# Chthi/Ofighters

Hardware: AMD Instinct MI355X
Metric: arena-steps/sec (env.step+obs+policy fwd) at 4096 arenas, 1/2/4/8 MI355X (higher is better)
Workload: dtype f32; 1 GPU; 4096 arenas x 8 ships per GPU, random-bot actions + step + 2D obs rasterise (u8 maps) + bi-head policy forward for 8 ship(s)/arena, trunk shared per arena (BASELINE configs[3]); arenas_per_gpu=4096, ships=8, laser_cap=512, episode_ticks=200, parallelism=arena-sharded x1, RCCL all-reduce of episodic scores only, laser_overflow=0, last_episode_score_sum=70993, last_episode_arenas=4096

## Files before the change

### ofighters_amd/csrc/ofx_head.hip

```cpp
#include "ofx_head.h"
#include "ofx_lowp.h"
#include "ofx_diag.h"
#include <stdlib.h>


typedef float f32x4 __attribute__((ext_vector_type(4)));
typedef float f32x2 __attribute__((ext_vector_type(2)));
#define HD_PS 400
constexpr int HC4_ZERO = 800;
constexpr int HC4_COL = 816, HC4_CPITCH = 416;
constexpr int HC4_STRIDE = HC4_COL + 2 * HC4_CPITCH + 16;
__device__ __forceinline__ int hc4_at(int ln, int t) { return ln < 2 ? ln * 400 + t : HC4_COL + (ln - 2) * HC4_CPITCH + t; }
__device__ __forceinline__ int hc4_pad(int k) { return k < 16 ? HC4_ZERO + k : k < 32 ? HC4_COL + 400 + k - 16 : HC4_COL + HC4_CPITCH + 400 + k - 32; }

__device__ __forceinline__ void hc4_zero_block(const HeadParams2 &p, int tid, int threads) {
  if (blockIdx.x == 0)
    for (int e = tid; e < HC4_STRIDE; e += threads) p.c4[(size_t)p.S * HC4_STRIDE + e] = 0.f;
}

__device__ __forceinline__ float hd_max_raw(float x, float floor) {
  float pinf;
  asm("s_mov_b32 %0, 0x7f800000" : "=s"(pinf));
  return __builtin_amdgcn_fmed3f(x, floor, pinf);
}
// ... 182 lines not shown
    float acc = 0.f;
    if (!isc || (t > 0 && t < 399)) {
      const int d0 = side ? 2 : 0;
#pragma unroll
      for (int d1 = 0; d1 < 3; d1++)
#pragma unroll
        for (int ci = 0; ci < 8; ci++) {
          const int tap = isc ? d1 * 3 + d0 : d0 * 3 + d1;
          acc += p.w4raw[tap * 8 + ci] * hf_up(u3l + ln * 1600 + ci, 8, 200, t + d1 - 1, p.legacy);
        }
      if (!isc && (t == 0 || t == 399)) {
        const int cl = t ? 3 : 2, dx = t ? 2 : 0;
        for (int dy = 0; dy < 3; dy++) {
          if (dy == d0) continue;
          const int yy = (side ? 399 : 0) + dy - 1;
          if (yy < 0 || yy > 399) continue;
          for (int ci = 0; ci < 8; ci++) acc += p.w4raw[(dy * 3 + dx) * 8 + ci] * hf_up(u3l + cl * 1600 + ci, 8, 200, yy, p.legacy);
        }
      }
    }
    p.c4[(size_t)s * HC4_STRIDE + hc4_at(ln, t)] = acc;
  }
  if (tid < 64) p.c4[(size_t)s * HC4_STRIDE + hc4_pad(tid)] = 0.f;
}

constexpr int HG_THREADS = 256;
constexpr int HG_L1 = 0;
constexpr int HG_U3 = 0;
constexpr int HG_RB = 6400;
constexpr int HG_CB = HG_RB + 4 * 102 * 4;
constexpr int HG_TOTAL = HG_CB + 4 * 102 * 4;
static_assert(2 * 52 * 52 <= 6400, "l1p fits under u3l");

template <int CIN, int COUT, class G>
__device__ __forceinline__ float hg_corner(G get, int n, int yc, int xc, const float *w, float bias, int co, int legacy) {
  float acc = bias;
  for (int dy = 0; dy < 3; dy++) {
    const int uy = yc + dy - 1;
    if (uy < 0 || uy >= 2 * n) continue;
    int ya, yb; float wy;
    hf_taps(uy, n, ya, yb, wy, legacy);
    for (int dx = 0; dx < 3; dx++) {
      const int ux = xc + dx - 1;
      if (ux < 0 || ux >= 2 * n) continue;
      int xa, xb; float wx;
      hf_taps(ux, n, xa, xb, wx, legacy);
      for (int ci = 0; ci < CIN; ci++) {
        const float a = get(ya, xa, ci), b = get(ya, xb, ci), d = get(yb, xa, ci), g = get(yb, xb, ci);
        const float top = a + (b - a) * wx, bot = d + (g - d) * wx;
        acc += w[((dy * 3 + dx) * CIN + ci) * COUT + co] * (top + (bot - top) * wy);
      }
    }
  }
  return fmaxf(acc, 0.f);
}

__global__ __launch_bounds__(HG_THREADS) void k_head_frames(HeadParams2 p) {
  __shared__ __align__(16) float sm[HG_TOTAL];
  __shared__ float efr_s[192], w4s[72];
  const int s = hd_ship(p, (int)((blockIdx.x & ~7u) | ((blockIdx.x + (blockIdx.x >> 3)) & 7u)));
  const int tid = threadIdx.x, lane = tid & 63;
  hc4_zero_block(p, tid, HG_THREADS);
  if (s < 0) return;
  const int wv = __builtin_amdgcn_readfirstlane(tid >> 6);
  const int n16 = lane & 15, kq = lane >> 4;
  float *l1p = sm + HG_L1, *u2rb = sm + HG_RB, *u2cb = sm + HG_CB, *u3l = sm + HG_U3;

  {
    constexpr int NB = 6 * 52 + 46 * 6, NE = 2 * NB, PER = (NE + HG_THREADS - 1) / HG_THREADS;
    float v[PER];
    int at[PER];
#pragma unroll
    for (int u = 0; u < PER; u++) {
      const int e = min(u * HG_THREADS + tid, NE - 1);
      const int ci = e / NB, k = e - ci * NB;
      int r, c;
      if (k < 6 * 52) { const int rr = k / 52; r = rr < 3 ? rr : rr + 46; c = k - rr * 52; }
      else { const int k2 = k - 6 * 52, cc = k2 % 6; r = 3 + k2 / 6; c = cc < 3 ? cc : cc + 46; }
      at[u] = (ci * 52 + r) * 52 + c;
      v[u] = p.up1[(size_t)s * 5000 + (ci * 50 + min(max(r - 1, 0), 49)) * 50 + min(max(c - 1, 0), 49)];
    }
#pragma unroll
    for (int u = 0; u < PER; u++)
      if (u * HG_THREADS + tid < NE) l1p[at[u]] = v[u];
  }
  if (tid < 192) efr_s[tid] = p.efr[tid];
  if (tid < 72) w4s[tid] = p.w4raw[tid];
  __syncthreads();

  float bw2[5];
#pragma unroll
  for (int jj = 0; jj < 5; jj++) bw2[jj] = p.w2fr[(wv * 20 + 4 * jj + kq) * 16 + n16];
  float bw3[9];
#pragma unroll
  for (int jj = 0; jj < 9; jj++) bw3[jj] = p.w3fr[(wv * 36 + 4 * jj + kq) * 16 + n16];
#pragma unroll 1
  for (int m = 0; m < 4; m++) {
    const int v = wv;
    const int pp = min(16 * m + n16, 49);
    const int i = v == 0 ? 0 : v == 1 ? 49 : pp, j = v == 2 ? 0 : v == 3 ? 49 : pp;
    const float bias = p.b2[n16 & 3];
    f32x4 d = {bias, bias, bias, bias};
#pragma unroll
    for (int jj = 0; jj < 5; jj++) {
      const int tap = min(2 * jj + (kq >> 1), 8);
      const float a = l1p[((kq & 1) * 52 + i + tap / 3) * 52 + j + tap % 3];
      d = __builtin_amdgcn_mfma_f32_16x16x4f32(a, bw2[jj], d, 0, 0, 0);
    }
    const int co = n16 & 3, pa = n16 >> 3, pb = (n16 >> 2) & 1;
#pragma unroll
    for (int r = 0; r < 4; r++) {
      const int q = 16 * m + 4 * kq + r;
      if (q >= 50) continue;
      const float val = fmaxf(d[r], 0.f);
      if (v < 2) {
        u2rb[((2 * v + pa) * 102 + 2 * q + pb + 1) * 4 + co] = val;
      } else {
        u2cb[((2 * (v - 2) + pb) * 102 + 2 * q + pa + 1) * 4 + co] = val;
      }
    }
  }
  __syncthreads();
  if (tid < 64) {
    const int co = tid & 3, cx = (tid >> 2) & 1, cy = (tid >> 3) & 1, bx = (tid >> 4) & 1, by = tid >> 5;
    const int y = by ? 98 + cy : cy, x = bx ? 98 + cx : cx;
    const int rb = by ? 2 + cy : cy, cb = bx ? 2 + cx : cx;
    const bool fy = y == 0 || y == 99, fx = x == 0 || x == 99;
    float val;
    if (fy && fx) {
      auto get = [&](int yy, int xx, int ci) { return l1p[(ci * 52 + yy + 1) * 52 + xx + 1]; };
      val = hg_corner<2, 4>(get, 50, y, x, p.w2raw, p.b2[co], co, p.legacy);
    } else if (fx) {
      val = u2cb[(cb * 102 + y + 1) * 4 + co];
    } else {
      val = u2rb[(rb * 102 + x + 1) * 4 + co];
    }
    if (fy && fx) { u2rb[(rb * 102 + x + 1) * 4 + co] = val; u2cb[(cb * 102 + y + 1) * 4 + co] = val; }
    else if (fx) u2rb[(rb * 102 + x + 1) * 4 + co] = val;
    else u2cb[(cb * 102 + y + 1) * 4 + co] = val;
  }
  __syncthreads();
  if (tid < 128) {
    const int co = tid & 3, b = (tid >> 2) & 3, hi = (tid >> 4) & 1, isc = tid >> 5;
    if (isc < 2) {
      float *ln = (isc ? u2cb : u2rb) + b * 102 * 4;
      ln[(hi ? 101 : 0) * 4 + co] = ln[(hi ? 100 : 1) * 4 + co];
    }
  }
  for (int e = tid; e < 4 * 100 * 4; e += HG_THREADS) {
    const int ln = e / 400, r = e - ln * 400;
    const float *src = ln < 2 ? u2rb + (ln ? 3 : 0) * 408 : u2cb + (ln == 3 ? 3 : 0) * 408;
    p.u2fr[(size_t)s * 1600 + e] = src[4 + r];
  }
  __syncthreads();

#pragma unroll 1
  for (int m = 0; m < 7; m++) {
    const int v = wv;
    const int qq = min(16 * m + n16, 99);
    const float *band = (v < 2 ? u2rb : u2cb);
    const int b0 = (v & 1) ? 2 : 0;
    const float bias = p.b3[n16 & 7];
    f32x4 d = {bias, bias, bias, bias};
#pragma unroll
    for (int jj = 0; jj < 9; jj++) {
      const int ty = jj / 3, tx = jj % 3;
      const int tf = v < 2 ? ty : tx, ta = v < 2 ? tx : ty;
      const int bsel = (v & 1) ? b0 + min(tf, 1) : b0 + max(tf - 1, 0);
      const float a = band[(bsel * 102 + qq + ta) * 4 + kq];
      d = __builtin_amdgcn_mfma_f32_16x16x4f32(a, bw3[jj], d, 0, 0, 0);
    }
    const int co = n16 & 7, par = n16 >> 3;
#pragma unroll
    for (int r = 0; r < 4; r++) {
      const int q = 16 * m + 4 * kq + r;
      if (q < 100) u3l[(v * 200 + 2 * q + par) * 8 + co] = fmaxf(d[r], 0.f);
    }
  }
  __syncthreads();
  if (tid < 32) {
    const int co = tid & 7, c = tid >> 3;
    const int y = (c & 1) ? 199 : 0, x = (c & 2) ? 199 : 0;
    auto get = [&](int yy, int xx, int ci) {
      return u2rb[((yy < 50 ? yy : yy - 96) * 102 + xx + 1) * 4 + ci];
    };
    const float val = hg_corner<4, 8>(get, 100, y, x, p.w3raw, p.b3[co], co, p.legacy);
    u3l[(((c & 1) ? 1 : 0) * 200 + x) * 8 + co] = val;
    u3l[(((c & 2) ? 3 : 2) * 200 + y) * 8 + co] = val;
  }
  __syncthreads();
  if (tid < 252) {
    const int tp = tid % 9, c0 = tid / 9;
    float wt[8];
#pragma unroll
    for (int ci = 0; ci < 8; ci++) wt[ci] = w4s[tp * 8 + ci];
    float *dst = p.vfr + (size_t)s * 7200 + tid;
    for (int cell = c0; cell < 4 * 200; cell += 28) {
      const f32x4 ua = *reinterpret_cast<const f32x4 *>(u3l + cell * 8), ub = *reinterpret_cast<const f32x4 *>(u3l + cell * 8 + 4);
      float acc = 0.f;
#pragma unroll
      for (int ci = 0; ci < 4; ci++) acc = fmaf(wt[ci], ua[ci], acc);
#pragma unroll
      for (int ci = 0; ci < 4; ci++) acc = fmaf(wt[4 + ci], ub[ci], acc);
      dst[(cell - c0) * 9] = acc;
    }
  }

  for (int e = tid; e < 4 * 400; e += HG_THREADS) {
    const int ln = e / 400, t = e - ln * 400, isc = ln >> 1, side = ln & 1, jq = t >> 1, b = t & 1;
    float acc = 0.f;
    if (!isc || (t > 0 && t < 399)) {
      const float *E = efr_s + ((isc * 2 + side) * 2 + b) * 24;
      const float *L = u3l + ln * 1600;
#pragma unroll
      for (int o = 0; o < 3; o++) {
        const float *Lp = L + min(max(jq + o - 1, 0), 199) * 8;
#pragma unroll
        for (int ci = 0; ci < 8; ci++) acc += E[o * 8 + ci] * Lp[ci];
      }
      if (!isc && (t == 0 || t == 399)) {
        const int cs = t ? 1 : 0;
        const int yq = side ? 199 : 0, a = side ? 1 : 0;
        const float *E2 = efr_s + ((2 + cs) * 2 + a) * 24;
        const float *L2 = u3l + (2 + cs) * 1600;
        for (int o = 0; o < 3; o++) {
          const float *Lp = L2 + min(max(yq + o - 1, 0), 199) * 8;
          for (int ci = 0; ci < 8; ci++) acc += E2[o * 8 + ci] * Lp[ci];
        }
        const int tap = (side ? 2 : 0) * 3 + (cs ? 2 : 0);
        const float *Lc = L + (t ? 199 : 0) * 8;
        for (int ci = 0; ci < 8; ci++) acc -= p.w4raw[tap * 8 + ci] * Lc[ci];
      }
    }
    p.c4[(size_t)s * HC4_STRIDE + hc4_at(ln, t)] = acc;
  }
  if (tid < 64) p.c4[(size_t)s * HC4_STRIDE + hc4_pad(tid)] = 0.f;
}

constexpr int HS_GPR = 13;
constexpr int HS_NTILES = 325;
constexpr int HS_NS = 42;
constexpr int HS_NR3 = 16, HS_P3 = 106;
constexpr int HS_PL3 = HS_NR3 * HS_P3 + 4;
constexpr int HS_NV = 9;
constexpr int HS_NR2 = 16, HS_P2 = 56;
constexpr int HS_PL2 = (HS_NR2 + 2) * HS_P2;
static_assert(HS_PL2 % 32 == 16, "uprelu2 plane stride");
constexpr int HS_TABP = 16 * HS_GPR;
static_assert(HS_TABP == 4 * 52, "table period in tiles");
static_assert(4 * (HS_NV * HS_PL3 + 4 * HS_PL2 + HS_TABP + 400) <= 80 * 1024, "two workgroups per CU");
struct alignas(16) HsPick { signed char v[HS_NS][4]; };
constexpr int hs_pairs_done_c(int s) { return s + 2 + ((s + 2) >> 2) < 50 ? s + 2 + ((s + 2) >> 2) : 50; }
constexpr HsPick hs_make_pick() {
  HsPick t{};
  for (int st = 0; st < HS_NS; st++)
    for (int cw = 0; cw < 4; cw++) {
      const int lo = 2 * hs_pairs_done_c(st), hi = 2 * hs_pairs_done_c(st + 1);
      const int at = lo + ((cw - lo) & 3);
      t.v[st][cw] = (signed char)(at < hi ? at >> 1 : -1);
    }
  return t;
}
__constant__ HsPick kHsPick = hs_make_pick();

__device__ __forceinline__ int hs_tiles_done(int s) {
  return s < 0 ? 0 : min(HS_NTILES, 8 * (s + 1) + ((s + 1) >> 3));
}
// ... 555 lines not shown
```

### ofighters_amd/csrc/ofx_policy.hip

```cpp
#include <string.h>

#include "ofx_internal.h"
#include "ofx_blob.h"
#include "ofx_trunk.h"
#include "ofx_head.h"

typedef float f32x16 __attribute__((ext_vector_type(16)));


extern "C" int ofx_policy_layout(const ofx_handle *h, ofx_policy_desc *desc) {
  (void)h;
  if (!desc) { ofx_set_error("ofx_policy_layout: null desc"); return OFX_ERR_INVALID; }
  memset(desc, 0, sizeof(*desc));
  desc->n_tensors = policy_layout(desc->offset, desc->count);
  desc->n_floats = desc->offset[desc->n_tensors];
  return OFX_OK;
}

struct PrepLayout {
  int tw[4], tb[4];
  int uw[3], ub[3];
  int w3mf;
  int w2mf;
  int w2fr;
  int w3fr;
  int w4eff_c;
  int w4raw;
  int efr;
  int b4;
  int zero16;
  int wbm[3];
  int lut1;
  int total;
};

static PrepLayout prep_layout() {
  PrepLayout L;
  int off = 0;
  for (int i = 0; i < 4; i++) { L.tw[i] = off; off += 9 * kTrunkCin[i] * 8; L.tb[i] = off; off += 8; }
  for (int i = 0; i < 3; i++) { L.uw[i] = off; off += 9 * kUpCin[i] * kUpCout[i]; L.ub[i] = off; off += kUpCout[i]; }
// ... 119 lines not shown
        for (int dy = 0; dy < 3; dy++)
          for (int dx = 0; dx < 3; dx++) {
            const bool drop = (v == 0 && a == 0 && dy == 0) || (v == 1 && a == 1 && dy == 2) || (v == 2 && b == 0 && dx == 0) ||
                              (v == 3 && b == 1 && dx == 2);
            if (!drop) acc += (p.w[p.src_k[5] + ((dy * 3 + dx) * 2 + ci) * 4 + co] * inv) * (up_coef(a, dy, ty, p.legacy) * up_coef(b, dx, tx, p.legacy));
          }
      }
      p.prep[p.dst_w2fr + e] = acc;
    }
    for (int e = tid; e < 4 * 36 * 16; e += nthr) {
      const int n = e % 16, k = (e / 16) % 36, v = e / 576, co = n & 7, q = n >> 3, ci = k & 3, tap = k >> 2;
      const int a = v == 0 ? 0 : v == 1 ? 1 : q, b = v == 2 ? 0 : v == 3 ? 1 : q, ty = tap / 3, tx = tap % 3;
      const float inv = g3[co] / sqrtf(g3[3 * 8 + co] + 1e-3f);
      float acc = 0.f;
      for (int dy = 0; dy < 3; dy++)
        for (int dx = 0; dx < 3; dx++) {
          const bool drop = (v == 0 && dy == 0) || (v == 1 && dy == 2) || (v == 2 && dx == 0) || (v == 3 && dx == 2);
          if (!drop) acc += (p.w[p.src_k[6] + ((dy * 3 + dx) * 4 + ci) * 8 + co] * inv) * (up_coef(a, dy, ty, p.legacy) * up_coef(b, dx, tx, p.legacy));
        }
      p.prep[p.dst_w3fr + e] = acc;
    }
  }
  if (tid == 0) p.prep[p.dst_b4] = p.w[p.src_b4];
  } else {
  for (int l = 1; l < 4; l++)
    for (int e = tid; e < 24 * 64; e += nthr) {
      const int lane = e & 63, j = e >> 6, n16 = lane & 15, kq = lane >> 4, co = n16 >> 1, r = n16 & 1;
      const int k = 4 * j + kq, rd = k >> 3, ci = k & 7, row = rd / 3, dx = rd - row * 3, tr = row - r;
      p.prep[p.dst_wbm[l - 1] + e] = (tr >= 0 && tr < 3) ? p.prep[p.dst_w[l] + ((tr * 3 + dx) * 8 + ci) * 8 + co] : 0.f;
    }
  }
}

__global__ __launch_bounds__(256) void k_upconv1(ConvParams p) {
  __shared__ float u0s[625];
  __shared__ float up[52][53];
  const int tid = threadIdx.x;
  const int n_items = p.live ? p.live[0] : p.images;
#pragma unroll 1
  for (int it = blockIdx.x; it < n_items; it += gridDim.x) {
  const int img = p.live ? p.live[1 + it] : it;
  __syncthreads();
  for (int e = tid; e < 625; e += 256) u0s[e] = p.in[(size_t)img * 625 + e];
  __syncthreads();
  for (int e = tid; e < 52 * 52; e += 256) {
    const int c = e % 52, r = e / 52, gy = r - 1, gx = c - 1;
    float v = 0.f;
    if (gy >= 0 && gy < 50 && gx >= 0 && gx < 50) {
      const float sy = p.legacy ? (float)gy * 0.5f : ((float)gy + 0.5f) * 0.5f - 0.5f;
      const float sx = p.legacy ? (float)gx * 0.5f : ((float)gx + 0.5f) * 0.5f - 0.5f;
      const float fy = floorf(sy), fx = floorf(sx);
      const float ly = sy - fy, lx = sx - fx;
      int y0 = (int)fy, x0 = (int)fx, y1 = y0 + 1, x1 = x0 + 1;
      y0 = max(y0, 0); x0 = max(x0, 0); y1 = min(y1, 24); x1 = min(x1, 24);
      const float a = u0s[y0 * 25 + x0], b = u0s[y0 * 25 + x1], d = u0s[y1 * 25 + x0], g = u0s[y1 * 25 + x1];
      const float top = a + (b - a) * lx, bot = d + (g - d) * lx;
      v = top + (bot - top) * ly;
    }
    up[r][c] = v;
  }
  __syncthreads();
  if (tid < 250) {
  const int row = tid / 5, x0 = 10 * (tid - 5 * row);
  float acc[2][10];
#pragma unroll
  for (int co = 0; co < 2; co++)
#pragma unroll
    for (int i = 0; i < 10; i++) acc[co][i] = 0.f;
#pragma unroll
  for (int dy = 0; dy < 3; dy++) {
    float v[12];
#pragma unroll
    for (int i = 0; i < 12; i++) v[i] = up[row + dy][x0 + i];
#pragma unroll
    for (int dx = 0; dx < 3; dx++)
#pragma unroll
      for (int co = 0; co < 2; co++) {
        const float wv = p.w[(dy * 3 + dx) * 2 + co];
#pragma unroll
        for (int i = 0; i < 10; i++) acc[co][i] = __builtin_fmaf(v[i + dx], wv, acc[co][i]);
      }
  }
#pragma unroll
  for (int co = 0; co < 2; co++) {
    const float bias = p.b[co];
    float *o = p.out + (((size_t)img * 2 + co) * 50 + row) * 50 + x0;
#pragma unroll
    for (int i = 0; i < 10; i += 2)
      *reinterpret_cast<float2 *>(o + i) = make_float2(fmaxf(acc[co][i] + bias, 0.f), fmaxf(acc[co][i + 1] + bias, 0.f));
  }
  }
  }
}


__global__ __launch_bounds__(256) void k_gemm_f32(const float *A, int lda, const float *B, int ldb, const float *bias,
                                                  float *C, int ldc, int M, int N, int K, int relu, const int32_t *live) {
  const int lane = threadIdx.x & 63, wv = threadIdx.x >> 6;
  const int tiles_n = (N + 31) / 32;
  const int tile = blockIdx.x * 4 + wv;
  if (live) M = live[0];
  if (tile >= ((M + 31) / 32) * tiles_n) return;
  const int m0 = (tile / tiles_n) * 32, n0 = (tile % tiles_n) * 32;
  const int r0 = m0 + (lane & 31), c = n0 + (lane & 31), kh = lane >> 5;
  const bool rv = r0 < M, cv = c < N;
  const int r = live ? live[1 + (rv ? r0 : 0)] : r0;
  f32x16 acc;
#pragma unroll
  for (int i = 0; i < 16; i++) acc[i] = 0.f;
  const float *ap = A + (size_t)(rv ? r : 0) * lda + kh;
  const float *bp = B + (size_t)kh * ldb + (cv ? c : 0);
  for (int k0 = 0; k0 < K; k0 += 2) {
    const bool kv = k0 + kh < K;
    const float a = (rv && kv) ? ap[k0] : 0.f;
    const float b = (cv && kv) ? bp[(size_t)k0 * ldb] : 0.f;
    acc = __builtin_amdgcn_mfma_f32_32x32x2f32(a, b, acc, 0, 0, 0);
  }
  if (cv) {
    const float bv = bias ? bias[c] : 0.f;
#pragma unroll
    for (int i = 0; i < 16; i++) {
      const int row = m0 + (i & 3) + 8 * (i >> 2) + 4 * kh;
      if (row < M) {
        float v = acc[i] + bv;
        if (relu) v = fmaxf(v, 0.f);
        C[(size_t)(live ? live[1 + row] : row) * ldc + c] = v;
      }
    }
  }
}

__global__ __launch_bounds__(256) void k_gemm_f32_splitk(const float *A, int lda, const float *B, int ldb, float *P,
                                                         int M, int N, int Kc, int tiles, int jobs) {
  const int lane = threadIdx.x & 63, wv = threadIdx.x >> 6;
  const int tiles_n = (N + 31) / 32;
  const int job = blockIdx.x * 4 + wv;
  const int chunk = job / tiles, tile = job - chunk * tiles;
  if (job >= jobs) return;
  const int m0 = (tile / tiles_n) * 32, n0 = (tile % tiles_n) * 32;
  const int r = m0 + (lane & 31), c = n0 + (lane & 31), kh = lane >> 5;
  const bool rv = r < M, cv = c < N;
  f32x16 acc;
#pragma unroll
  for (int i = 0; i < 16; i++) acc[i] = 0.f;
  const float *ap = A + (size_t)(rv ? r : 0) * lda + (size_t)chunk * Kc + 4 * kh;
  const float *bp = B + ((size_t)chunk * Kc + 4 * kh) * ldb + (cv ? c : 0);
  for (int k0 = 0; k0 < Kc; k0 += 8) {
    const float4 a4 = *reinterpret_cast<const float4 *>(ap + k0);
    const float b0 = bp[(size_t)(k0 + 0) * ldb], b1 = bp[(size_t)(k0 + 1) * ldb], b2 = bp[(size_t)(k0 + 2) * ldb],
                b3 = bp[(size_t)(k0 + 3) * ldb];
    acc = __builtin_amdgcn_mfma_f32_32x32x2f32(rv ? a4.x : 0.f, cv ? b0 : 0.f, acc, 0, 0, 0);
    acc = __builtin_amdgcn_mfma_f32_32x32x2f32(rv ? a4.y : 0.f, cv ? b1 : 0.f, acc, 0, 0, 0);
    acc = __builtin_amdgcn_mfma_f32_32x32x2f32(rv ? a4.z : 0.f, cv ? b2 : 0.f, acc, 0, 0, 0);
    acc = __builtin_amdgcn_mfma_f32_32x32x2f32(rv ? a4.w : 0.f, cv ? b3 : 0.f, acc, 0, 0, 0);
  }
  if (cv) {
    float *out = P + (size_t)chunk * M * N;
#pragma unroll
    for (int i = 0; i < 16; i++) {
      const int row = m0 + (i & 3) + 8 * (i >> 2) + 4 * kh;
      if (row < M) out[(size_t)row * N + c] = acc[i];
    }
  }
}

struct HeadParams {
  int N, M;
  ofx_state st;
  const float *g1;
  int g1_chunks;
  const float *k1, *b1, *k2, *b2, *k3, *b3;
  const int32_t *live;
  const uint8_t *mask;
  const float *vec8;
  float *d1;
  float *act;
  int32_t *iaction;
};

__global__ __launch_bounds__(256) void k_head_dense(HeadParams p) {
  __shared__ float sd1[4][100];
  __shared__ float sd2[4][50];
  const int lane = threadIdx.x & 63, wv = threadIdx.x >> 6;
  const int item = blockIdx.x * 4 + wv, n_items = p.live ? p.live[0] : p.N * p.M;
  if ((int)blockIdx.x * 4 >= n_items) return;
  const bool on = item < n_items;
  const int s = on ? (p.live ? p.live[1 + item] : item) : 0;
// ... 70 lines not shown

struct PolicyWs {
  float *p1, *p2, *p3, *p4, *g1, *d1, *u0, *up1, *u2fr, *vfr, *c4;
  unsigned long long *best;
  int32_t *iaction, *ipointer, *live;
};

static size_t al(size_t b) { return (b + 255) & ~(size_t)255; }
constexpr int kDense1Chunks = 25;

static int policy_workspace(ofx_handle *h, PolicyWs *ws, size_t N, size_t S) {
  size_t f2, f3, f4;
  ofx_head_frame_bytes(S, &f2, &f3, &f4);
  const size_t sz[] = {ofx_trunk_fused(h, N) ? 0 : al(4ull * N * 8 * 200 * 200), al(4ull * N * 8 * 100 * 100), al(4ull * N * 8 * 50 * 50),
                       al(4ull * N * 5000),          al(4ull * N * 100 * kDense1Chunks), al(4ull * S * 100),
                       al(4ull * S * 625),           al(4ull * S * 2 * 50 * 50),   al(f2), al(f3), al(f4),
                       al(8ull * S),                 al(4ull * S),                 al(8ull * S),
                       al(4ull * (S + 1))};
  size_t total = 0;
  for (size_t b : sz) total += b;
  int rc = ofx_ensure_scratch(h, total);
  if (rc) return rc;
  char *base = (char *)h->scratch;
  void **dst[] = {(void **)&ws->p1,   (void **)&ws->p2,   (void **)&ws->p3,      (void **)&ws->p4,      (void **)&ws->g1,
                  (void **)&ws->d1,   (void **)&ws->u0,   (void **)&ws->up1,     (void **)&ws->u2fr,    (void **)&ws->vfr,
                  (void **)&ws->c4,   (void **)&ws->best, (void **)&ws->iaction, (void **)&ws->ipointer,
                  (void **)&ws->live};
  for (size_t i = 0; i < sizeof(sz) / sizeof(sz[0]); i++) { *dst[i] = base; base += sz[i]; }
  return OFX_OK;
}

int ofx_launch_gemm(ofx_handle *h, const float *A, int lda, const float *B, int ldb, const float *bias, float *C, int ldc,
                    int M, int N, int K, int relu, const int32_t *live) {
  const int tiles = ((M + 31) / 32) * ((N + 31) / 32);
  hipLaunchKernelGGL(k_gemm_f32, dim3((tiles + 3) / 4), dim3(256), 0, h->stream, A, lda, B, ldb, bias, C, ldc, M, N, K,
                     relu, live);
  OFX_HIP(hipGetLastError());
  return OFX_OK;
}

static int policy_prepare(ofx_handle *h, const float *weights, float **slot) {
  const PrepLayout L = prep_layout();
  if (!*slot) {
    OFX_HIP(hipMalloc((void **)slot, sizeof(float) * L.total));
    OFX_HIP(hipMemsetAsync(*slot, 0, sizeof(float) * L.total, h->stream));
  }
  int32_t off[64], cnt[64];
  policy_layout(off, cnt);
  PrepParams pp;
  pp.w = weights; pp.prep = *slot;
  for (int i = 0; i < 4; i++) {
    pp.src_k[i] = off[ofx_t_trunk(i)]; pp.src_b[i] = off[ofx_t_trunk(i, OFX_T_BIAS)]; pp.src_g[i] = off[ofx_t_trunk(i, OFX_T_GAMMA)];
    pp.cin[i] = kTrunkCin[i]; pp.cout[i] = 8; pp.dst_w[i] = L.tw[i]; pp.dst_b[i] = L.tb[i];
  }
  for (int i = 0; i < 3; i++) {
    pp.src_k[4 + i] = off[ofx_t_up(i)]; pp.src_b[4 + i] = off[ofx_t_up(i, OFX_T_BIAS)]; pp.src_g[4 + i] = off[ofx_t_up(i, OFX_T_GAMMA)];
    pp.cin[4 + i] = kUpCin[i]; pp.cout[4 + i] = kUpCout[i]; pp.dst_w[4 + i] = L.uw[i]; pp.dst_b[4 + i] = L.ub[i];
  }
  pp.src_k4 = off[OFX_T_OUT2]; pp.src_b4 = off[OFX_T_OUT2 + 1];
  pp.dst_w4raw = L.w4raw; pp.dst_b4 = L.b4; pp.dst_efr = L.efr;
  pp.dst_w4eff_c = L.w4eff_c; pp.dst_w3mf = L.w3mf; pp.dst_w2mf = L.w2mf; pp.dst_w2fr = L.w2fr; pp.dst_w3fr = L.w3fr; pp.dst_lut1 = L.lut1;
  for (int i = 0; i < 3; i++) pp.dst_wbm[i] = L.wbm[i];
  pp.legacy = h->opt_bilinear_legacy;
  pp.phase = 0;
  hipLaunchKernelGGL(k_policy_prepare, dim3(32), dim3(256), 0, h->stream, pp);
  pp.phase = 1;
  hipLaunchKernelGGL(k_policy_prepare, dim3(4), dim3(256), 0, h->stream, pp);
  OFX_HIP(hipGetLastError());
  return OFX_OK;
// ... 53 lines not shown
  float *act_values, *heatmap, *ptr_max, *ptr_probe;
  int32_t *iaction, *ipointer;
  const int32_t *probe;
};

static int policy_forward_impl(ofx_handle *h, const ForwardArgs &a) {
  const int N = a.N, S = a.N * a.M;
  const float *weights = a.weights;
  PolicyWs ws;
  int rc = policy_workspace(h, &ws, N, S);
  if (rc) return rc;
  int32_t off[64], cnt[64];
  policy_layout(off, cnt);
  const PrepLayout L = prep_layout();

  const bool pinned = h->prep && h->prep_pinned == weights;
  if (!pinned && (rc = policy_prepare(h, weights, &h->prep_tmp))) return rc;
  const float *prep = pinned ? h->prep : h->prep_tmp;

  const int lowp = a.vec8 == nullptr ? h->opt_policy_lowp : 0;
  TrunkParams tp;
  memset(&tp, 0, sizeof(tp));
  tp.bits[0] = a.bits[0]; tp.bits[1] = a.bits[1]; tp.bits_stride = a.bits_stride; tp.images = N;
  for (int i = 0; i < 4; i++) { tp.tw[i] = prep + L.tw[i]; tp.tb[i] = prep + L.tb[i]; }
  for (int i = 0; i < 3; i++) tp.wbm[i] = prep + L.wbm[i];
  tp.lut1 = prep + L.lut1; tp.zero16 = prep + L.zero16;
  tp.p1 = ws.p1; tp.p2 = ws.p2; tp.p3 = ws.p3; tp.p4 = ws.p4;
  tp.lowp = lowp; tp.sparse = !h->opt_trunk_dense || a.vec8 != nullptr;
  tp.stat = h->opt_trunk_count ? h->trunk_stat : nullptr;
  if ((rc = ofx_launch_trunk(h, tp))) return rc;

  const float *k1 = weights + off[OFX_T_DENSE1];
  {
    const int tiles = ((N + 31) / 32) * 4, jobs = tiles * kDense1Chunks;
    hipLaunchKernelGGL(k_gemm_f32_splitk, dim3((jobs + 3) / 4), dim3(256), 0, h->stream, ws.p4, 5000, k1 + 8 * 100, 100,
                       ws.g1, N, 100, 5000 / kDense1Chunks, tiles, jobs);
    OFX_HIP(hipGetLastError());
  }
  HeadParams hp;
  hp.N = N; hp.M = a.M; hp.st = h->st; hp.vec8 = a.vec8; hp.g1 = ws.g1; hp.g1_chunks = kDense1Chunks;
  hp.k1 = k1; hp.b1 = weights + off[OFX_T_DENSE1 + 1];
  hp.k2 = weights + off[OFX_T_DENSE2]; hp.b2 = weights + off[OFX_T_DENSE2 + 1];
  hp.k3 = weights + off[OFX_T_OUT1]; hp.b3 = weights + off[OFX_T_OUT1 + 1];
  const int32_t *live = nullptr;
  if (a.ship_mask) {
    if ((rc = ofx_head_compact(h, S, a.ship_mask, ws.live))) return rc;
    live = ws.live;
  }
  hp.mask = a.ship_mask; hp.live = live; hp.d1 = ws.d1; hp.act = a.act_values; hp.iaction = a.iaction ? a.iaction : ws.iaction;
  hipLaunchKernelGGL(k_head_dense, dim3((S + 3) / 4), dim3(256), 0, h->stream, hp);
  OFX_HIP(hipGetLastError());

  if ((rc = ofx_launch_gemm(h, ws.d1, 100, weights + off[OFX_T_UPDENSE], 625, weights + off[OFX_T_UPDENSE + 1], ws.u0, 625, S, 625, 100, 1, live)))
    return rc;
  ConvParams up;
  memset(&up, 0, sizeof(up));
  up.live = live; up.images = S; up.legacy = h->opt_bilinear_legacy;
  up.in = ws.u0; up.w = prep + L.uw[0]; up.b = prep + L.ub[0]; up.out = ws.up1;
  hipLaunchKernelGGL(k_upconv1, dim3((unsigned)(live && S > 4096 ? 4096 : S)), dim3(256), 0, h->stream, up);
  OFX_HIP(hipGetLastError());
  OFX_HIP(hipMemsetAsync(ws.best, 0, sizeof(unsigned long long) * S, h->stream));
  HeadParams2 hp2;
  memset(&hp2, 0, sizeof(hp2));
  hp2.S = S; hp2.up1 = ws.up1;
  hp2.w2mf = prep + L.w2mf; hp2.b2 = prep + L.ub[1]; hp2.w2raw = prep + L.uw[1];
  hp2.w3mf = prep + L.w3mf; hp2.b3 = prep + L.ub[2]; hp2.w3raw = prep + L.uw[2];
  hp2.w4eff_c = prep + L.w4eff_c; hp2.b4 = prep + L.b4; hp2.w4raw = prep + L.w4raw;
  hp2.w2fr = prep + L.w2fr; hp2.w3fr = prep + L.w3fr; hp2.efr = prep + L.efr;
  hp2.u2fr = ws.u2fr; hp2.vfr = ws.vfr; hp2.c4 = ws.c4;
  hp2.frames_ref = h->opt_frames_ref; hp2.legacy = h->opt_bilinear_legacy;
  hp2.bf16 = lowp;
  hp2.mask = a.ship_mask; hp2.live = ws.live; hp2.live_ready = a.ship_mask != nullptr; hp2.best = ws.best; hp2.heat = a.heatmap;
  hp2.probe = a.probe; hp2.ptr_probe = a.probe ? a.ptr_probe : nullptr;
  const int pb = h->prof_base;
  hp2.event_base = pb;
  if ((rc = ofx_launch_head(h, hp2))) return rc;
  if (pb >= 0) h->prof_base = pb + 3 < OFX_RING_MAX ? pb + 2 : -1;
  hipLaunchKernelGGL(k_policy_finish, dim3((S + 255) / 256), dim3(256), 0, h->stream, S, a.ship_mask, ws.best,
                     a.ipointer ? a.ipointer : ws.ipointer, a.ptr_max);
  OFX_HIP(hipGetLastError());
  return OFX_OK;
}

static int live_forward_check(ofx_handle *h, const float *weights, const char *who) {
  if (!h || !weights) { ofx_set_error("%s: null argument", who); return OFX_ERR_INVALID; }
  if (!h->spawned) { ofx_set_error("You must execute analyse_battleground first."); return OFX_ERR_STATE; }
  const ofx_config &c = h->cfg;
  if (c.width != PS || c.height != PS) {
    ofx_set_error("%s: the pointer_model takes 400x400 maps (got %d x %d)", who, c.width, c.height);
    return OFX_ERR_INVALID;
  }
  return OFX_OK;
// ... 237 lines not shown
```

Baseline: 227,300 arena-steps/s.

## Rework head frames, upconv1 and dense GEMMs with LDS-staged weights and precomputed indices

In k_head_frames, the halo gather indices move into a constexpr __constant__ table, weight loads are hoisted before the first barrier, corner-conv weights are preloaded into registers, and the per-element copy and c4 loops are remapped to one wave per line with vector LDS reads. k_upconv1 is templated on the legacy flag, does separable bilinear upsampling from registers instead of an LDS u0 copy, and stages its output in LDS so global stores are float4. The split-K dense1 GEMM and a new K=100 GEMM stage the B tile in LDS and prefetch A rows in batches, replacing strided per-lane B global loads. The aim is less address arithmetic, fewer scattered global accesses and more overlap of loads with compute. In exchange, LDS use and register pressure rise, which could reduce occupancy.

Measured after the change: 229,900 arena-steps/s, median of 6. 1.01x the previous value.

```diff
diff --git a/ofighters_amd/csrc/ofx_head.hip b/ofighters_amd/csrc/ofx_head.hip
--- a/ofighters_amd/csrc/ofx_head.hip
+++ b/ofighters_amd/csrc/ofx_head.hip
@@ -238,28 +238,53 @@
 constexpr int HG_TOTAL = HG_CB + 4 * 102 * 4;
 static_assert(2 * 52 * 52 <= 6400, "l1p fits under u3l");
 
-template <int CIN, int COUT, class G>
-__device__ __forceinline__ float hg_corner(G get, int n, int yc, int xc, const float *w, float bias, int co, int legacy) {
+template <int CIN, int COUT>
+__device__ __forceinline__ void hg_corner_w(const float *w, int yc, int xc, int co, float (&wr)[4 * CIN]) {
+  const int dy0 = yc == 0 ? 1 : 0, dx0 = xc == 0 ? 1 : 0;
+#pragma unroll
+  for (int t = 0; t < 4; t++)
+#pragma unroll
+    for (int ci = 0; ci < CIN; ci++) wr[t * CIN + ci] = w[(((dy0 + (t >> 1)) * 3 + dx0 + (t & 1)) * CIN + ci) * COUT + co];
+}
+template <int CIN, class G>
+__device__ __forceinline__ float hg_corner(G get, int n, int yc, int xc, const float (&wr)[4 * CIN], float bias, int legacy) {
   float acc = bias;
-  for (int dy = 0; dy < 3; dy++) {
-    const int uy = yc + dy - 1;
-    if (uy < 0 || uy >= 2 * n) continue;
+  const int dy0 = yc == 0 ? 1 : 0, dx0 = xc == 0 ? 1 : 0;
+#pragma unroll
+  for (int a2 = 0; a2 < 2; a2++) {
     int ya, yb; float wy;
-    hf_taps(uy, n, ya, yb, wy, legacy);
-    for (int dx = 0; dx < 3; dx++) {
-      const int ux = xc + dx - 1;
-      if (ux < 0 || ux >= 2 * n) continue;
+    hf_taps(yc + dy0 + a2 - 1, n, ya, yb, wy, legacy);
+#pragma unroll
+    for (int b2 = 0; b2 < 2; b2++) {
       int xa, xb; float wx;
-      hf_taps(ux, n, xa, xb, wx, legacy);
+      hf_taps(xc + dx0 + b2 - 1, n, xa, xb, wx, legacy);
+#pragma unroll
       for (int ci = 0; ci < CIN; ci++) {
         const float a = get(ya, xa, ci), b = get(ya, xb, ci), d = get(yb, xa, ci), g = get(yb, xb, ci);
         const float top = a + (b - a) * wx, bot = d + (g - d) * wx;
-        acc += w[((dy * 3 + dx) * CIN + ci) * COUT + co] * (top + (bot - top) * wy);
+        acc += wr[(a2 * 2 + b2) * CIN + ci] * (top + (bot - top) * wy);
       }
     }
   }
   return fmaxf(acc, 0.f);
 }
+
+constexpr int HG_NB = 6 * 52 + 46 * 6, HG_NE = 2 * HG_NB, HG_PER = (HG_NE + HG_THREADS - 1) / HG_THREADS;
+struct alignas(16) HgStage { unsigned v[HG_PER * HG_THREADS]; };
+constexpr HgStage hg_make_stage() {
+  HgStage t{};
+  for (int e0 = 0; e0 < HG_PER * HG_THREADS; e0++) {
+    const int e = e0 < HG_NE ? e0 : HG_NE - 1;
+    const int ci = e / HG_NB, k = e - ci * HG_NB;
+    int r = 0, c = 0;
+    if (k < 6 * 52) { const int rr = k / 52; r = rr < 3 ? rr : rr + 46; c = k - rr * 52; }
+    else { const int k2 = k - 6 * 52, cc = k2 % 6; r = 3 + k2 / 6; c = cc < 3 ? cc : cc + 46; }
+    const int rs = r - 1 < 0 ? 0 : r - 1 > 49 ? 49 : r - 1, cs = c - 1 < 0 ? 0 : c - 1 > 49 ? 49 : c - 1;
+    t.v[e0] = (unsigned)((ci * 52 + r) * 52 + c) | (unsigned)((ci * 50 + rs) * 50 + cs) << 16;
+  }
+  return t;
+}
+__constant__ HgStage kHgStage = hg_make_stage();
 
 __global__ __launch_bounds__(HG_THREADS) void k_head_frames(HeadParams2 p) {
   __shared__ __align__(16) float sm[HG_TOTAL];
@@ -272,40 +297,42 @@
   const int n16 = lane & 15, kq = lane >> 4;
   float *l1p = sm + HG_L1, *u2rb = sm + HG_RB, *u2cb = sm + HG_CB, *u3l = sm + HG_U3;
 
-  {
-    constexpr int NB = 6 * 52 + 46 * 6, NE = 2 * NB, PER = (NE + HG_THREADS - 1) / HG_THREADS;
-    float v[PER];
-    int at[PER];
-#pragma unroll
-    for (int u = 0; u < PER; u++) {
-      const int e = min(u * HG_THREADS + tid, NE - 1);
-      const int ci = e / NB, k = e - ci * NB;
-      int r, c;
-      if (k < 6 * 52) { const int rr = k / 52; r = rr < 3 ? rr : rr + 46; c = k - rr * 52; }
-      else { const int k2 = k - 6 * 52, cc = k2 % 6; r = 3 + k2 / 6; c = cc < 3 ? cc : cc + 46; }
-      at[u] = (ci * 52 + r) * 52 + c;
-      v[u] = p.up1[(size_t)s * 5000 + (ci * 50 + min(max(r - 1, 0), 49)) * 50 + min(max(c - 1, 0), 49)];
-    }
-#pragma unroll
-    for (int u = 0; u < PER; u++)
-      if (u * HG_THREADS + tid < NE) l1p[at[u]] = v[u];
-  }
-  if (tid < 192) efr_s[tid] = p.efr[tid];
-  if (tid < 72) w4s[tid] = p.w4raw[tid];
-  __syncthreads();
-
+  constexpr int NE = HG_NE, PER = HG_PER;
+  unsigned at[PER];
+#pragma unroll
+  for (int u = 0; u < PER; u++) at[u] = kHgStage.v[u * HG_THREADS + tid];
+  const float efr_v = p.efr[min(tid, 191)], w4_v = p.w4raw[min(tid, 71)];
   float bw2[5];
 #pragma unroll
   for (int jj = 0; jj < 5; jj++) bw2[jj] = p.w2fr[(wv * 20 + 4 * jj + kq) * 16 + n16];
   float bw3[9];
 #pragma unroll
   for (int jj = 0; jj < 9; jj++) bw3[jj] = p.w3fr[(wv * 36 + 4 * jj + kq) * 16 + n16];
+  const float b2v = p.b2[n16 & 3], b3v = p.b3[n16 & 7];
+  float wc2[8], wc3[16];
+  if (wv == 0) {
+    hg_corner_w<2, 4>(p.w2raw, (lane >> 5) ? 99 : 0, ((lane >> 4) & 1) ? 99 : 0, lane & 3, wc2);
+    hg_corner_w<4, 8>(p.w3raw, ((lane >> 3) & 1) ? 199 : 0, ((lane >> 3) & 2) ? 199 : 0, lane & 7, wc3);
+  }
+  {
+    float v[PER];
+    const float *src = p.up1 + (size_t)s * 5000;
+#pragma unroll
+    for (int u = 0; u < PER; u++) v[u] = src[at[u] >> 16];
+#pragma unroll
+    for (int u = 0; u < PER; u++)
+      if (u * HG_THREADS + tid < NE) l1p[at[u] & 0xFFFFu] = v[u];
+  }
+  if (tid < 192) efr_s[tid] = efr_v;
+  if (tid < 72) w4s[tid] = w4_v;
+  __syncthreads();
+
 #pragma unroll 1
   for (int m = 0; m < 4; m++) {
     const int v = wv;
     const int pp = min(16 * m + n16, 49);
     const int i = v == 0 ? 0 : v == 1 ? 49 : pp, j = v == 2 ? 0 : v == 3 ? 49 : pp;
-    const float bias = p.b2[n16 & 3];
+    const float bias = b2v;
     f32x4 d = {bias, bias, bias, bias};
 #pragma unroll
     for (int jj = 0; jj < 5; jj++) {
@@ -335,7 +362,7 @@
     float val;
     if (fy && fx) {
       auto get = [&](int yy, int xx, int ci) { return l1p[(ci * 52 + yy + 1) * 52 + xx + 1]; };
-      val = hg_corner<2, 4>(get, 50, y, x, p.w2raw, p.b2[co], co, p.legacy);
+      val = hg_corner<2>(get, 50, y, x, wc2, b2v, p.legacy);
     } else if (fx) {
       val = u2cb[(cb * 102 + y + 1) * 4 + co];
     } else {
@@ -353,10 +380,14 @@
       ln[(hi ? 101 : 0) * 4 + co] = ln[(hi ? 100 : 1) * 4 + co];
     }
   }
-  for (int e = tid; e < 4 * 100 * 4; e += HG_THREADS) {
-    const int ln = e / 400, r = e - ln * 400;
-    const float *src = ln < 2 ? u2rb + (ln ? 3 : 0) * 408 : u2cb + (ln == 3 ? 3 : 0) * 408;
-    p.u2fr[(size_t)s * 1600 + e] = src[4 + r];
+  {
+    const float *src = (wv < 2 ? u2rb : u2cb) + ((wv & 1) ? 3 : 0) * 408 + 4;
+    float *dst = p.u2fr + (size_t)s * 1600 + wv * 400;
+#pragma unroll
+    for (int k = 0; k < 7; k++) {
+      const int r = lane + 64 * k;
+      if (r < 400) dst[r] = src[r];
+    }
   }
   __syncthreads();
 
@@ -366,7 +397,7 @@
     const int qq = min(16 * m + n16, 99);
     const float *band = (v < 2 ? u2rb : u2cb);
     const int b0 = (v & 1) ? 2 : 0;
-    const float bias = p.b3[n16 & 7];
+    const float bias = b3v;
     f32x4 d = {bias, bias, bias, bias};
 #pragma unroll
     for (int jj = 0; jj < 9; jj++) {
@@ -390,7 +421,7 @@
     auto get = [&](int yy, int xx, int ci) {
       return u2rb[((yy < 50 ? yy : yy - 96) * 102 + xx + 1) * 4 + ci];
     };
-    const float val = hg_corner<4, 8>(get, 100, y, x, p.w3raw, p.b3[co], co, p.legacy);
+    const float val = hg_corner<4>(get, 100, y, x, wc3, b3v, p.legacy);
     u3l[(((c & 1) ? 1 : 0) * 200 + x) * 8 + co] = val;
     u3l[(((c & 2) ? 3 : 2) * 200 + y) * 8 + co] = val;
   }
@@ -412,18 +443,27 @@
     }
   }
 
-  for (int e = tid; e < 4 * 400; e += HG_THREADS) {
-    const int ln = e / 400, t = e - ln * 400, isc = ln >> 1, side = ln & 1, jq = t >> 1, b = t & 1;
-    float acc = 0.f;
-    if (!isc || (t > 0 && t < 399)) {
-      const float *E = efr_s + ((isc * 2 + side) * 2 + b) * 24;
-      const float *L = u3l + ln * 1600;
+  {
+    const int ln = wv, isc = ln >> 1, side = ln & 1;
+    const float *L = u3l + ln * 1600;
+    float E[24];
+#pragma unroll
+    for (int i = 0; i < 24; i++) E[i] = efr_s[(ln * 2 + (lane & 1)) * 24 + i];
+    float *dst = p.c4 + (size_t)s * HC4_STRIDE + hc4_at(ln, 0);
+#pragma unroll 1
+    for (int k = 0; k < 7; k++) {
+      const int t = lane + 64 * k, jq = t >> 1;
+      float acc = 0.f;
 #pragma unroll
       for (int o = 0; o < 3; o++) {
         const float *Lp = L + min(max(jq + o - 1, 0), 199) * 8;
-#pragma unroll
-        for (int ci = 0; ci < 8; ci++) acc += E[o * 8 + ci] * Lp[ci];
-      }
+        const f32x4 la = *reinterpret_cast<const f32x4 *>(Lp), lb = *reinterpret_cast<const f32x4 *>(Lp + 4);
+#pragma unroll
+        for (int ci = 0; ci < 4; ci++) acc += E[o * 8 + ci] * la[ci];
+#pragma unroll
+        for (int ci = 0; ci < 4; ci++) acc += E[o * 8 + 4 + ci] * lb[ci];
+      }
+      if (isc && (t == 0 || t == 399)) acc = 0.f;
       if (!isc && (t == 0 || t == 399)) {
         const int cs = t ? 1 : 0;
         const int yq = side ? 199 : 0, a = side ? 1 : 0;
@@ -435,10 +475,10 @@
         }
         const int tap = (side ? 2 : 0) * 3 + (cs ? 2 : 0);
         const float *Lc = L + (t ? 199 : 0) * 8;
-        for (int ci = 0; ci < 8; ci++) acc -= p.w4raw[tap * 8 + ci] * Lc[ci];
-      }
-    }
-    p.c4[(size_t)s * HC4_STRIDE + hc4_at(ln, t)] = acc;
+        for (int ci = 0; ci < 8; ci++) acc -= w4s[tap * 8 + ci] * Lc[ci];
+      }
+      if (t < 400) dst[t] = acc;
+    }
   }
   if (tid < 64) p.c4[(size_t)s * HC4_STRIDE + hc4_pad(tid)] = 0.f;
 }
diff --git a/ofighters_amd/csrc/ofx_policy.hip b/ofighters_amd/csrc/ofx_policy.hip
--- a/ofighters_amd/csrc/ofx_policy.hip
+++ b/ofighters_amd/csrc/ofx_policy.hip
@@ -6,6 +6,7 @@
 #include "ofx_head.h"
 
 typedef float f32x16 __attribute__((ext_vector_type(16)));
+typedef float f32x4 __attribute__((ext_vector_type(4)));
 
 
 extern "C" int ofx_policy_layout(const ofx_handle *h, ofx_policy_desc *desc) {
@@ -191,32 +192,51 @@
   }
 }
 
+template <bool LEGACY>
 __global__ __launch_bounds__(256) void k_upconv1(ConvParams p) {
-  __shared__ float u0s[625];
   __shared__ float up[52][53];
+  __shared__ __align__(16) float outs[5000];
   const int tid = threadIdx.x;
+  const int seg = tid / 52, c = tid - 52 * seg;
+  const int R = 13 * seg + (seg & 1), K = R >> 1, nrow = 14 - 2 * (seg & 1);
+  const int gx = c - 1, kx = gx >> 1, oddx = gx & 1;
+  const bool colv = gx >= 0 && gx < 50;
+  const int xa = min(max(LEGACY ? kx : kx - 1 + oddx, 0), 24), xb = min(max(LEGACY ? kx + 1 : kx + oddx, 0), 24);
+  const float lx = LEGACY ? (oddx ? 0.5f : 0.f) : (oddx ? 0.25f : 0.75f);
+  constexpr int nt = LEGACY ? 9 : 8;
   const int n_items = p.live ? p.live[0] : p.images;
 #pragma unroll 1
   for (int it = blockIdx.x; it < n_items; it += gridDim.x) {
   const int img = p.live ? p.live[1 + it] : it;
+  float t[9];
+  if (tid < 208) {
+    const float *src = p.in + (size_t)img * 625;
+    float a[9], b[9];
+#pragma unroll
+    for (int i = 0; i < 9; i++)
+      if (i < nt) {
+        const unsigned y25 = 25u * (unsigned)min(max(K - 1 + i, 0), 24);
+        a[i] = src[y25 + (unsigned)xa];
+        b[i] = src[y25 + (unsigned)xb];
+      }
+#pragma unroll
+    for (int i = 0; i < 9; i++) t[i] = i < nt ? a[i] + (b[i] - a[i]) * lx : 0.f;
+  }
   __syncthreads();
-  for (int e = tid; e < 625; e += 256) u0s[e] = p.in[(size_t)img * 625 + e];
-  __syncthreads();
-  for (int e = tid; e < 52 * 52; e += 256) {
-    const int c = e % 52, r = e / 52, gy = r - 1, gx = c - 1;
-    float v = 0.f;
-    if (gy >= 0 && gy < 50 && gx >= 0 && gx < 50) {
-      const float sy = p.legacy ? (float)gy * 0.5f : ((float)gy + 0.5f) * 0.5f - 0.5f;
-      const float sx = p.legacy ? (float)gx * 0.5f : ((float)gx + 0.5f) * 0.5f - 0.5f;
-      const float fy = floorf(sy), fx = floorf(sx);
-      const float ly = sy - fy, lx = sx - fx;
-      int y0 = (int)fy, x0 = (int)fx, y1 = y0 + 1, x1 = x0 + 1;
-      y0 = max(y0, 0); x0 = max(x0, 0); y1 = min(y1, 24); x1 = min(x1, 24);
-      const float a = u0s[y0 * 25 + x0], b = u0s[y0 * 25 + x1], d = u0s[y1 * 25 + x0], g = u0s[y1 * 25 + x1];
-      const float top = a + (b - a) * lx, bot = d + (g - d) * lx;
-      v = top + (bot - top) * ly;
-    }
-    up[r][c] = v;
+  if (tid < 208) {
+#pragma unroll
+    for (int j = 0; j < 14; j++) {
+      const int m = j >> 1, r = R + j;
+      float v;
+      if constexpr (LEGACY) {
+        const float top = t[m + (j & 1)], bot = t[m + (j & 1) + 1];
+        v = top + (bot - top) * ((j & 1) ? 0.f : 0.5f);
+      } else {
+        const float top = t[m], bot = t[m + 1];
+        v = top + (bot - top) * ((j & 1) ? 0.75f : 0.25f);
+      }
+      if (j < nrow) up[r][c] = (colv && r >= 1 && r <= 50) ? v : 0.f;
+    }
   }
   __syncthreads();
   if (tid < 250) {
@@ -243,12 +263,15 @@
 #pragma unroll
   for (int co = 0; co < 2; co++) {
     const float bias = p.b[co];
-    float *o = p.out + (((size_t)img * 2 + co) * 50 + row) * 50 + x0;
+    float *o = outs + (co * 50 + row) * 50 + x0;
 #pragma unroll
     for (int i = 0; i < 10; i += 2)
       *reinterpret_cast<float2 *>(o + i) = make_float2(fmaxf(acc[co][i] + bias, 0.f), fmaxf(acc[co][i + 1] + bias, 0.f));
   }
   }
+  __syncthreads();
+  for (int e = tid; e < 1250; e += 256)
+    *reinterpret_cast<float4 *>(p.out + (size_t)img * 5000 + 4 * e) = *reinterpret_cast<const float4 *>(outs + 4 * e);
   }
 }
 
@@ -289,29 +312,123 @@
   }
 }
 
+__global__ __launch_bounds__(256) void k_gemm_f32_k100(const float *A, int lda, const float *B, int ldb, const float *bias,
+                                                       float *C, int ldc, int M, int N, int relu, const int32_t *live,
+                                                       int tiles_n) {
+  constexpr int K = 100, NT = K / 2, NQ = (NT + 3) / 4;
+  __shared__ __align__(16) float bs[NQ * 2 * 32 * 4];
+  const int tid = threadIdx.x, lane = tid & 63, wv = __builtin_amdgcn_readfirstlane(tid >> 6);
+  const int nt = blockIdx.x % tiles_n, mg = blockIdx.x / tiles_n;
+  if (live) M = live[0];
+  if (mg * 128 >= M) return;
+  const int m0 = (mg * 4 + wv) * 32, n0 = nt * 32;
+  const int r0 = m0 + (lane & 31), c = n0 + (lane & 31), kh = lane >> 5;
+  const bool rv = r0 < M, cv = c < N;
+  {
+    const float *bp = B + (n0 + (tid & 31) < N ? n0 + (tid & 31) : 0);
+    f32x4 w[(2 * NQ + 7) / 8];
+#pragma unroll
+    for (int i = 0; i < (2 * NQ + 7) / 8; i++) {
+      const int gk = min((tid >> 5) + 8 * i, 2 * NQ - 1), q = gk >> 1, h = gk & 1;
+#pragma unroll
+      for (int j = 0; j < 4; j++) w[i][j] = bp[(size_t)(2 * min(4 * q + j, NT - 1) + h) * ldb];
+    }
+#pragma unroll
+    for (int i = 0; i < (2 * NQ + 7) / 8; i++) {
+      const int gk = (tid >> 5) + 8 * i;
+      if (gk < 2 * NQ) *reinterpret_cast<f32x4 *>(bs + (gk * 32 + (tid & 31)) * 4) = w[i];
+    }
+  }
+  const int r = live ? live[1 + (rv ? r0 : 0)] : (rv ? r0 : 0);
+  const float *ap = A + (size_t)r * lda;
+  constexpr int NU = K / 4, NB0 = 9, NB1 = 8;
+  f32x4 a[NU];
+#pragma unroll
+  for (int u = 0; u < NB0; u++) a[u] = *reinterpret_cast<const f32x4 *>(ap + 4 * u);
+  __syncthreads();
+  if (m0 >= M) return;
+  f32x16 acc;
+#pragma unroll
+  for (int i = 0; i < 16; i++) acc[i] = 0.f;
+  const float *bl = bs + (kh * 32 + (lane & 31)) * 4;
+  f32x4 b4[NQ];
+#pragma unroll
+  for (int u = 0; u < NU; u++) {
+    if (u == 0) {
+#pragma unroll
+      for (int i = NB0; i < NB0 + NB1; i++) a[i] = *reinterpret_cast<const f32x4 *>(ap + 4 * i);
+    }
+    if (u == NB0) {
+#pragma unroll
+      for (int i = NB0 + NB1; i < NU; i++) a[i] = *reinterpret_cast<const f32x4 *>(ap + 4 * i);
+    }
+    if ((u & 1) == 0) b4[u >> 1] = *reinterpret_cast<const f32x4 *>(bl + (u >> 1) * 2 * 32 * 4);
+    acc = __builtin_amdgcn_mfma_f32_32x32x2f32(kh ? a[u][1] : a[u][0], b4[u >> 1][(2 * u) & 3], acc, 0, 0, 0);
+    acc = __builtin_amdgcn_mfma_f32_32x32x2f32(kh ? a[u][3] : a[u][2], b4[u >> 1][(2 * u + 1) & 3], acc, 0, 0, 0);
+  }
+  if (cv) {
+    const float bv = bias ? bias[c] : 0.f;
+#pragma unroll
+    for (int i = 0; i < 16; i++) {
+      const int row = m0 + (i & 3) + 8 * (i >> 2) + 4 * kh;
+      if (row < M) {
+        float v = acc[i] + bv;
+        if (relu) v = fmaxf(v, 0.f);
+        C[(size_t)(live ? live[1 + row] : row) * ldc + c] = v;
+      }
+    }
+  }
+}
+
+constexpr int kSplitKc = 200;
 __global__ __launch_bounds__(256) void k_gemm_f32_splitk(const float *A, int lda, const float *B, int ldb, float *P,
-                                                         int M, int N, int Kc, int tiles, int jobs) {
-  const int lane = threadIdx.x & 63, wv = threadIdx.x >> 6;
-  const int tiles_n = (N + 31) / 32;
-  const int job = blockIdx.x * 4 + wv;
-  const int chunk = job / tiles, tile = job - chunk * tiles;
-  if (job >= jobs) return;
-  const int m0 = (tile / tiles_n) * 32, n0 = (tile % tiles_n) * 32;
+                                                         int M, int N, int tiles_n, int groups_m) {
+  constexpr int Kc = kSplitKc, KG = Kc / 4, STEPS = Kc / 8;
+  __shared__ __align__(16) float bs[KG * 32 * 4];
+  const int tid = threadIdx.x, lane = tid & 63, wv = __builtin_amdgcn_readfirstlane(tid >> 6);
+  const int nt = blockIdx.x % tiles_n, rest = blockIdx.x / tiles_n, mg = rest % groups_m, chunk = rest / groups_m;
+  const int m0 = (mg * 4 + wv) * 32, n0 = nt * 32;
   const int r = m0 + (lane & 31), c = n0 + (lane & 31), kh = lane >> 5;
   const bool rv = r < M, cv = c < N;
+  {
+    const float *bp = B + (size_t)chunk * Kc * ldb + (n0 + (tid & 31) < N ? n0 + (tid & 31) : 0);
+    f32x4 w[(KG + 7) / 8];
+#pragma unroll
+    for (int i = 0; i < (KG + 7) / 8; i++) {
+      const int g = min((tid >> 5) + 8 * i, KG - 1);
+#pragma unroll
+      for (int j = 0; j < 4; j++) w[i][j] = bp[(size_t)(4 * g + j) * ldb];
+    }
+#pragma unroll
+    for (int i = 0; i < (KG + 7) / 8; i++) {
+      const int g = (tid >> 5) + 8 * i;
+      if (g < KG) *reinterpret_cast<f32x4 *>(bs + (g * 32 + (tid & 31)) * 4) = w[i];
+    }
+  }
+  const float *ap = A + (size_t)(rv ? r : 0) * lda + (size_t)chunk * Kc + 4 * kh;
+  constexpr int NB0 = 9, NB1 = 8;
+  f32x4 a[STEPS];
+#pragma unroll
+  for (int i = 0; i < NB0; i++) a[i] = *reinterpret_cast<const f32x4 *>(ap + 8 * i);
+  __syncthreads();
+  if (m0 >= M) return;
   f32x16 acc;
 #pragma unroll
   for (int i = 0; i < 16; i++) acc[i] = 0.f;
-  const float *ap = A + (size_t)(rv ? r : 0) * lda + (size_t)chunk * Kc + 4 * kh;
-  const float *bp = B + ((size_t)chunk * Kc + 4 * kh) * ldb + (cv ? c : 0);
-  for (int k0 = 0; k0 < Kc; k0 += 8) {
-    const float4 a4 = *reinterpret_cast<const float4 *>(ap + k0);
-    const float b0 = bp[(size_t)(k0 + 0) * ldb], b1 = bp[(size_t)(k0 + 1) * ldb], b2 = bp[(size_t)(k0 + 2) * ldb],
-                b3 = bp[(size_t)(k0 + 3) * ldb];
-    acc = __builtin_amdgcn_mfma_f32_32x32x2f32(rv ? a4.x : 0.f, cv ? b0 : 0.f, acc, 0, 0, 0);
-    acc = __builtin_amdgcn_mfma_f32_32x32x2f32(rv ? a4.y : 0.f, cv ? b1 : 0.f, acc, 0, 0, 0);
-    acc = __builtin_amdgcn_mfma_f32_32x32x2f32(rv ? a4.z : 0.f, cv ? b2 : 0.f, acc, 0, 0, 0);
-    acc = __builtin_amdgcn_mfma_f32_32x32x2f32(rv ? a4.w : 0.f, cv ? b3 : 0.f, acc, 0, 0, 0);
+  const float *bl = bs + (kh * 32 + (lane & 31)) * 4;
+#pragma unroll
+  for (int s = 0; s < STEPS; s++) {
+    if (s == 0) {
+#pragma unroll
+      for (int i = NB0; i < NB0 + NB1; i++) a[i] = *reinterpret_cast<const f32x4 *>(ap + 8 * i);
+    }
+    if (s == NB0) {
+#pragma unroll
+      for (int i = NB0 + NB1; i < STEPS; i++) a[i] = *reinterpret_cast<const f32x4 *>(ap + 8 * i);
+    }
+    const f32x4 b4 = *reinterpret_cast<const f32x4 *>(bl + s * 2 * 32 * 4);
+#pragma unroll
+    for (int j = 0; j < 4; j++) acc = __builtin_amdgcn_mfma_f32_32x32x2f32(a[s][j], b4[j], acc, 0, 0, 0);
   }
   if (cv) {
     float *out = P + (size_t)chunk * M * N;
@@ -448,9 +565,13 @@
 
 int ofx_launch_gemm(ofx_handle *h, const float *A, int lda, const float *B, int ldb, const float *bias, float *C, int ldc,
                     int M, int N, int K, int relu, const int32_t *live) {
-  const int tiles = ((M + 31) / 32) * ((N + 31) / 32);
-  hipLaunchKernelGGL(k_gemm_f32, dim3((tiles + 3) / 4), dim3(256), 0, h->stream, A, lda, B, ldb, bias, C, ldc, M, N, K,
-                     relu, live);
+  const int tiles_m = (M + 31) / 32, tiles_n = (N + 31) / 32, tiles = tiles_m * tiles_n;
+  if (K == 100 && lda % 4 == 0 && ((uintptr_t)A & 15) == 0)
+    hipLaunchKernelGGL(k_gemm_f32_k100, dim3((unsigned)(((tiles_m + 3) / 4) * tiles_n)), dim3(256), 0, h->stream, A, lda, B, ldb,
+                       bias, C, ldc, M, N, relu, live, tiles_n);
+  else
+    hipLaunchKernelGGL(k_gemm_f32, dim3((tiles + 3) / 4), dim3(256), 0, h->stream, A, lda, B, ldb, bias, C, ldc, M, N, K,
+                       relu, live);
   OFX_HIP(hipGetLastError());
   return OFX_OK;
 }
@@ -570,9 +691,10 @@
 
   const float *k1 = weights + off[OFX_T_DENSE1];
   {
-    const int tiles = ((N + 31) / 32) * 4, jobs = tiles * kDense1Chunks;
-    hipLaunchKernelGGL(k_gemm_f32_splitk, dim3((jobs + 3) / 4), dim3(256), 0, h->stream, ws.p4, 5000, k1 + 8 * 100, 100,
-                       ws.g1, N, 100, 5000 / kDense1Chunks, tiles, jobs);
+    static_assert(5000 == kDense1Chunks * kSplitKc, "k_gemm_f32_splitk's chunk");
+    const int tiles_n = (100 + 31) / 32, groups_m = ((N + 31) / 32 + 3) / 4;
+    hipLaunchKernelGGL(k_gemm_f32_splitk, dim3((unsigned)(tiles_n * groups_m * kDense1Chunks)), dim3(256), 0, h->stream, ws.p4,
+                       5000, k1 + 8 * 100, 100, ws.g1, N, 100, tiles_n, groups_m);
     OFX_HIP(hipGetLastError());
   }
   HeadParams hp;
@@ -595,7 +717,8 @@
   memset(&up, 0, sizeof(up));
   up.live = live; up.images = S; up.legacy = h->opt_bilinear_legacy;
   up.in = ws.u0; up.w = prep + L.uw[0]; up.b = prep + L.ub[0]; up.out = ws.up1;
-  hipLaunchKernelGGL(k_upconv1, dim3((unsigned)(live && S > 4096 ? 4096 : S)), dim3(256), 0, h->stream, up);
+  if (up.legacy) hipLaunchKernelGGL(k_upconv1<true>, dim3((unsigned)(live && S > 4096 ? 4096 : S)), dim3(256), 0, h->stream, up);
+  else hipLaunchKernelGGL(k_upconv1<false>, dim3((unsigned)(live && S > 4096 ? 4096 : S)), dim3(256), 0, h->stream, up);
   OFX_HIP(hipGetLastError());
   OFX_HIP(hipMemsetAsync(ws.best, 0, sizeof(unsigned long long) * S, h->stream));
   HeadParams2 hp2;
```
